# SensorsINI/v2e

Hardware: AMD Instinct MI355X
Metric: Mevents/s (EventEmulator.generate_events, 346x260, 10x slowdown) (higher is better)
Workload: dtype f64

## Files before the change

v2e_amd/csrc/emu_chain.h:

```cpp
#pragma once
#include <type_traits>
#include "pull_index.h"

#ifndef V2E_CHAIN_LOCKSTEP
#define V2E_CHAIN_LOCKSTEP 0
#endif
#ifndef V2E_CHAIN_STAMPS
#define V2E_CHAIN_STAMPS 0
#endif

constexpr int CHAIN_K_MAX = 64;
constexpr int CFRAME_THREADS = 1024;
constexpr int CHAIN_SUB = 8;
constexpr int CHAIN_MAX_ITERS = 1024;

template <typename R> __device__ __forceinline__ R floor_div_pos(R a, R b)
{
    if (!(b > (R)0) || !(a >= (R)0)) return div_floor<R>(a, b);
    if (a < b) return (R)0;
    R q = floor(a / b);
    R r = fma(-q, b, a);
    if (r < (R)0) q -= (R)1;
    else if (r >= b) q += (R)1;
    return q;
}

__device__ __forceinline__ bool clip_barrier(unsigned *ctr, unsigned target, bool light = false)
{
    __shared__ int s_ok;
    asm volatile("s_waitcnt vmcnt(0)" ::: "memory");
    __syncthreads();
    if (threadIdx.x == 0) {
        if (!light) {
            __builtin_amdgcn_fence(__ATOMIC_RELEASE, "agent");
            asm volatile("s_waitcnt vmcnt(0)" ::: "memory");
        }
        __hip_atomic_fetch_add(ctr, 1u, __ATOMIC_RELAXED, __HIP_MEMORY_SCOPE_AGENT);
        unsigned spins = 0;
        int ok = 1;
        while (__hip_atomic_load(ctr, __ATOMIC_RELAXED, __HIP_MEMORY_SCOPE_AGENT) < target) {
            if (light) __builtin_amdgcn_s_sleep(1); else __builtin_amdgcn_s_sleep(4);
            if (++spins > 2000000u) { ok = 0; break; }
        }
        if (!light) __builtin_amdgcn_fence(__ATOMIC_ACQUIRE, "agent");
        s_ok = ok;
    }
    __syncthreads();
    return s_ok != 0;
}

struct FrameTab {
    float start, step, end;
    uint32_t refr_mask;
    __device__ __forceinline__ FrameTab(const FrameCtl *c, int lane)
        : start(c->ts_start[lane & 31]), step(c->ts_stepf[lane & 31]), end(c->ts_end), refr_mask(c->refr_mask) {}
};

__device__ __forceinline__ TsGen frame_tsgen(const KArgs &a, const FrameCtl *c, const FrameTab &ft, int n, bool &use_refr)
{
    if (n <= 32) {
        use_refr = a.has_refr && ((ft.refr_mask >> (n - 1)) & 1u);
        return TsGen(__uint_as_float(lane_value(__float_as_uint(ft.start), n - 1)), ft.end,
                     __uint_as_float(lane_value(__float_as_uint(ft.step), n - 1)), n);
    }
    const double t_prev = c->t_prev, t_frame = c->t_frame;
    use_refr = a.has_refr && a.refr > (t_frame - t_prev) / (double)n;
    FrameCtl cc;
    cc.t_prev = t_prev; cc.t_frame = t_frame;
    return TsGen(cc, n, nullptr);
}

typedef float v2e_f4 __attribute__((ext_vector_type(4)));
typedef unsigned int v2e_u4 __attribute__((ext_vector_type(4)));
typedef unsigned int v2e_u2 __attribute__((ext_vector_type(2)));

__device__ __forceinline__ double lane_value_d(double v, int idx)
{
    const unsigned long long u = (unsigned long long)__double_as_longlong(v);
    return __longlong_as_double((long long)(((unsigned long long)lane_value((uint32_t)(u >> 32), idx) << 32) | lane_value((uint32_t)u, idx)));
}
__device__ __forceinline__ void store_event_wt(float4 *ev_clip, unsigned long long row, float t, float x, float y, float pol)
{
    if (row < 0x7000000ull) {
        const __amdgpu_buffer_rsrc_t r = __builtin_amdgcn_make_buffer_rsrc((void *)ev_clip, 0, 0x7fffffff, 0x00020000);
        const v2e_f4 v = {t, x, y, pol};
        __builtin_amdgcn_raw_buffer_store_b128(v, r, (int)(row * 16ull), 0, 17);
    } else {
        ev_clip[row] = make_float4(t, x, y, pol);
    }
}

struct ChainArgs {
    const void *const *frames_pp;
    unsigned long long frame_stride;
    const uint32_t *fidx_base;
    const FrameCtl *ctl;
    int f0, nf;
    int pf0, pnf;
    int D, n_clips, K, ngroups;
    int slot_f0, slot_pf0;
    uint32_t *cnt;
    uint32_t *ruleM;
    float *tsold;
    const uint2 *rec;
    uint32_t *gM_prev, *gM_cur;
    unsigned *bar_prev;
    const void *base_in, *lp_in;
    const float *ts_in;
    void *base_out, *lp_out;
    float *ts_out;
    const void *base_pin, *lp_pin;
    const float *ts_pin;
    void *base_fix, *lp_fix;
    float *ts_fix;
    void *ckc_base, *ckc_lp;
    float *ckc_ts;
    void *ckp_base, *ckp_lp;
    float *ckp_ts;
    v2e_frame_rec *recs;
    int store_out;
    int prio;
    int bar_light;
    int lockstep;
    unsigned long long *dbg;
    unsigned long long *const *stamp_pp;
    int lidx;
};

#define WT_STORE(ptr, val) __hip_atomic_store((ptr), (val), __ATOMIC_RELAXED, __HIP_MEMORY_SCOPE_SYSTEM)

#define V2E_STAMP_C(i) do { if (V2E_CHAIN_STAMPS && ca.dbg && tid == 0) ca.dbg[(size_t)g * 16 + (i)] = wall_clock64(); } while (0)

template <typename FT>
__device__ __forceinline__ void frame_record_table(const KArgs &a, FT px, const float *s_lutL, const double *s_lutI, double dt_over_tau,
                                                   double &L, double &inten01, double &eps)
{
    constexpr bool U8 = sizeof(FT) == 1;
    if (U8) {
        L = a.log_input ? (double)px : (double)s_lutL[(int)px];
        inten01 = s_lutI[(int)px];
    } else {
        const double x = (double)px;
        L = a.log_input ? x : (double)lin_log(x);
        inten01 = a.use_inten ? (x + 20.0) / 275.0 : 0.0;
    }
    eps = 0.0;
    if (a.has_cutoff) {
        eps = inten01 * dt_over_tau;
        if (eps > 1.0) eps = 1.0;
    }
}

__device__ __forceinline__ void frame_record_rand(const KArgs &a, double inten01, double shot_base, float dtime_f, float lk, float thp,
                                                  float ppre, float npre, float rr, float uu, float &dl, uint32_t &sb)
{
    dl = 0.f;
    if (a.do_leak) {
        const float rate = lk * (1.0f - a.jit_f * rr);
        dl = (dtime_f * rate) * thp;
    }
    sb = 0;
    if (a.do_shot) {
        const double F = shot_base * (a.inten_slope * inten01 + 1);
        if ((double)uu > 1 - F * (double)ppre) sb |= 1u;
        if ((double)uu < F * (double)npre) sb |= 2u;
    }
}

__device__ __forceinline__ uint4 pack_frame_record(double eps, double L, uint32_t dl_bits, uint32_t sb)
{
    const unsigned long long eb = (unsigned long long)__double_as_longlong(eps);
    uint4 r;
    r.x = (uint32_t)eb;
    r.y = (uint32_t)(eb >> 32) | (sb << 30);
    r.z = __float_as_uint((float)L);
    r.w = dl_bits;
    return r;
}

template <typename FT>
__device__ __forceinline__ uint4 make_frame_record(const KArgs &a, FT px, const float *s_lutL, const double *s_lutI, double dt_over_tau,
                                                   double shot_base, float dtime_f, float lk, float thp, float ppre, float npre, float rr,
                                                   float uu)
{
    double L, inten01, eps;
    frame_record_table<FT>(a, px, s_lutL, s_lutI, dt_over_tau, L, inten01, eps);
    float dl;
    uint32_t sb;
    frame_record_rand(a, inten01, shot_base, dtime_f, lk, thp, ppre, npre, rr, uu, dl, sb);
    return pack_frame_record(eps, L, __float_as_uint(dl), sb);
}

__device__ __forceinline__ uint4 decode_frame_record(const KArgs &a, uint2 r8, const float *s_lutL, const double *s_lutI, double dt_over_tau)
{
    const int px = (int)(r8.y & 0xFFu);
    const float tl = s_lutL[px];
    const double inten01 = s_lutI[px];
    const double L = a.log_input ? (double)px : (double)tl;
    double eps = 0.0;
    if (a.has_cutoff) {
        eps = inten01 * dt_over_tau;
        if (eps > 1.0) eps = 1.0;
    }
    return pack_frame_record(eps, L, r8.x, r8.y >> 30);
}

struct AheadArgs {
    const void *const *frames_pp;
    unsigned long long frame_stride;
    const FrameCtl *ctl;
    const uint32_t *fidx_base;
    int f0, nf, D, n_clips;
    int slot0;
    int ppt;
    uint2 *rec;
};

template <typename FT>
__global__ __launch_bounds__(BLOCK) void k_ahead(KArgs a, AheadArgs aa)
{
    static_assert(sizeof(FT) == 1, "k_ahead's records carry the pixel byte: uint8 frames only");
    __shared__ double s_lutI[256];
    const int tid = threadIdx.x;
    s_lutI[tid] = a.lut_I[tid];
    __syncthreads();
    const int clip = blockIdx.y, p = blockIdx.x * BLOCK + tid;
    if (p >= a.npx) return;
    const uint32_t fbase = *aa.fidx_base;
    const char *const frames = (const char *)*aa.frames_pp;
    const size_t sp = (size_t)clip * a.npx_pad + p;
    const bool need_r = a.do_leak && a.jit_f != 0.f;
    const float thp = a.pos_thres[sp], thn = a.neg_thres[sp];
    const float lk = a.do_leak ? a.leak_hz_f * a.noise_rate[sp] : 0.f;
    const float ppre = a.scalar_thres ? a.pos_pre_scalar : a.pos_nom_f / thp;
    const float npre = a.scalar_thres ? a.neg_pre_scalar : a.neg_nom_f / thn;
    v2e_philox_keys ks;
    v2e_philox_key_schedule((uint32_t)a.seed, (uint32_t)(a.seed >> 32), &ks);
    for (int zz = 0; zz < aa.ppt; ++zz) {
        const uint32_t q = v2e_frame_pair(fbase + (uint32_t)aa.f0) + blockIdx.z * (uint32_t)aa.ppt + (uint32_t)zz;
        const int f_odd = (int)(2u * q - 1u - fbase);
        const bool in0 = f_odd >= aa.f0 && f_odd < aa.f0 + aa.nf, in1 = f_odd + 1 >= aa.f0 && f_odd + 1 < aa.f0 + aa.nf;
        if (!in0 && !in1) continue;
        float r_odd = 0.f, u_odd = 0.f, r_even = 0.f, u_even = 0.f;
        if (need_r || a.do_shot) v2e_draw_pair_ks(&ks, (uint32_t)clip, q, (uint32_t)p, need_r, &r_odd, &u_odd, &r_even, &u_even);
#pragma unroll
        for (int half = 0; half < 2; ++half) {
            if (!(half ? in1 : in0)) continue;
            const int f = f_odd + half;
            int sl = aa.slot0 + (f - aa.f0);
            if (sl >= aa.D) sl -= aa.D;
            const FrameCtl *c = aa.ctl + (f * aa.n_clips + clip);
            const FT px = ((const FT *)(frames + (size_t)f * aa.frame_stride))[(size_t)clip * a.npx + p];
            float dl;
            uint32_t sb;
            frame_record_rand(a, s_lutI[px], c->shot_base, (float)(c->t_frame - c->t_prev), lk, thp, ppre, npre, half ? r_even : r_odd,
                              half ? u_even : u_odd, dl, sb);
            aa.rec[((uint32_t)sl * (uint32_t)aa.n_clips + (uint32_t)clip) * (uint32_t)a.npx_pad + (uint32_t)p] =
                make_uint2(__float_as_uint(dl), (uint32_t)px | (sb << 30));
        }
    }
}

template <typename R> __device__ __forceinline__ R floor_div_rcp(R a, R b, R rb)
{
    R q = floor(a * rb);
    R r = fma(-q, b, a);
    const bool lo = r < (R)0, hi = r >= b;
    q = lo ? q - (R)1 : (hi ? q + (R)1 : q);
    r = lo ? r + b : (hi ? r - b : r);
    if (__builtin_expect(!(r >= (R)0 && r < b), 0)) return floor_div_pos<R>(a, b);
    return q;
}

template <typename R, typename FT, bool FUSED, bool ALLON = false>
__global__ __launch_bounds__(BLOCK)
__attribute__((amdgpu_waves_per_eu((FUSED && sizeof(R) == 8 && sizeof(FT) == 1) ? 5 : (FUSED ? 1 : 2), 8)))
void k_chain(KArgs a_in, ChainArgs ca)
{
    KArgs a = a_in;
    if (ALLON) { a.has_cutoff = 1; a.do_leak = 1; a.do_shot = 1; a.has_refr = 1; a.use_inten = 1; }
    __shared__ float s_lutL[256];
    __shared__ double s_lutI[256];
    __shared__ double s_dtau[FUSED ? CHAIN_K_MAX : 1], s_shot[FUSED ? CHAIN_K_MAX : 1];
    __shared__ float s_dtime[FUSED ? CHAIN_K_MAX : 1];
    constexpr bool U8 = sizeof(FT) == 1;
    const int tid = threadIdx.x, lane = tid & (WAVE - 1);
    const int g = blockIdx.x;
    const int p = g * BLOCK + tid;
    const bool valid = p < a.npx;
    if (ca.prio) __builtin_amdgcn_s_setprio(3);
    V2E_STAMP_C(0);
    unsigned long long *const stamp = *ca.stamp_pp;
    if (stamp && tid == 0) atomicMax(stamp + 2 * ca.lidx, ~wall_clock64());
    uint32_t fbase = 0u;
    const char *frames = nullptr;
    float tab_L = 0.f;
    double tab_I = 0.0;
    if (!FUSED) {
        tab_L = a.lut_L[tid];
        tab_I = a.lut_I[tid];
    }
    if (FUSED) {
        fbase = *ca.fidx_base;
        frames = (const char *)*ca.frames_pp;
        if (U8) {
// ... 764 lines not shown
            uint32_t lane_tot = 0;
#pragma unroll
            for (int j = 0; j < 16; ++j) lane_tot += v[j];
            uint32_t run = carry + wave_excl_scan_u32(lane_tot, lane);
            carry += wave_sum_u32(lane_tot);
            if (wi < hi) {
                uint32_t o[16];
#pragma unroll
                for (int j = 0; j < 16; ++j) { o[j] = run; run += v[j]; }
                uint4 *dst = (uint4 *)(pre + (size_t)k * ea.nwp + wi);
                if (ea.cpre16) ea.cpre16[(((size_t)z * ea.n_clips + clip) * a.nkeys_cap + k) * (ea.nwp / 16) + wi / 16] = o[0];
                dst[0] = make_uint4(o[0], o[1], o[2], o[3]);
                dst[1] = make_uint4(o[4], o[5], o[6], o[7]);
                dst[2] = make_uint4(o[8], o[9], o[10], o[11]);
                dst[3] = make_uint4(o[12], o[13], o[14], o[15]);
            }
        }
        if (tid == 0) cT[k] = total;
    }
    __syncthreads();
    if (tid == 0) {
        __builtin_amdgcn_fence(__ATOMIC_RELEASE, "agent");
        const unsigned old = __hip_atomic_fetch_add(ea.cdone + zc, 1u, __ATOMIC_RELAXED, __HIP_MEMORY_SCOPE_AGENT);
        s_last = old == gridDim.x - 1;
        if (s_last) {
            __builtin_amdgcn_fence(__ATOMIC_ACQUIRE, "agent");
            __hip_atomic_store(ea.cdone + zc, 0u, __ATOMIC_RELAXED, __HIP_MEMORY_SCOPE_AGENT);
        }
    }
    __syncthreads();
    if (!s_last) return;
    if (discard) {
        if (tid == 0) {
            cf->M = M; cf->n_events = 0u; cf->n_signal = 0u; cf->discarded = 1u;
            rec->max_events = M;
            atomicOr(&rec->flags, V2E_FLAG_ITERS_CLAMPED);
        }
        return;
    }
    for (int k = tid; k < nk; k += CFRAME_THREADS) s_T[k] = __hip_atomic_load(cT + k, __ATOMIC_RELAXED, __HIP_MEMORY_SCOPE_AGENT);
    __syncthreads();
    if (wave != 0) return;
    uint32_t *ckb = ea.ckbase + zc * a.nkeys_cap;
    uint32_t carry = 0, sum_on = 0, sum_off = 0;
    for (int kb = 0; kb < nk; kb += WAVE) {
        const int key = kb + lane;
        const uint32_t T_k = key < nk ? s_T[key] : 0u;
        const uint32_t sig = key >= 2 ? T_k : 0u;
        const uint32_t kbase = carry + wave_excl_scan_u32(sig, lane);
        if (key < nk) ckb[key] = kbase;
        sum_on += wave_sum_u32((lane & 1) ? 0u : sig);
        sum_off += wave_sum_u32((lane & 1) ? sig : 0u);
        carry += wave_sum_u32(sig);
    }
    const uint32_t n_signal = carry;
    uint32_t *perm = ea.cperm + zc * a.max_iters * 8;
    if (a.shuffle && a.rng_mode == V2E_RNG_PHILOX) {
        const uint32_t fbase = ea.fidx_base ? *ea.fidx_base : 0u;
        for (int i = lane; i < M; i += WAVE) {
            uint32_t pk[4], sh, aa, amask;
            const uint32_t n_i = s_T[2 + 2 * i] + s_T[3 + 2 * i];
            v2e_perm_shape(n_i, &sh, &aa, &amask);
            v2e_perm_keys(a.seed, (uint32_t)clip, fbase + (uint32_t)fe, (uint32_t)i, pk);
            uint4 *pp = (uint4 *)(perm + (size_t)i * 8);
            pp[0] = make_uint4(pk[0], pk[1], pk[2], pk[3]);
            pp[1] = make_uint4(sh, aa, amask, n_i);
        }
    }
    if (lane == 0) {
        const uint32_t son = a.do_shot ? s_T[0] : 0u, soff = a.do_shot ? s_T[1] : 0u;
        cf->M = M; cf->n_signal = n_signal; cf->n_events = n_signal + son + soff; cf->discarded = 0u;
        rec->max_events = M;
        rec->n_signal = n_signal;
        rec->n_events = n_signal + son + soff;
        rec->n_on = sum_on + son;
        rec->n_off = sum_off + soff;
    }
}

__global__ __launch_bounds__(WAVE) void k_coff(CEmitArgs ea)
{
    const int clip = blockIdx.x, lane = threadIdx.x;
    unsigned long long tot = 0;
    for (int z = lane; z < ea.nE; z += WAVE) tot += ea.cf[(size_t)z * ea.n_clips + clip].n_events;
    const uint32_t lo = wave_sum_u32((uint32_t)(tot & 0xFFFFFFu)), hi = wave_sum_u32((uint32_t)(tot >> 24));
    if (lane == 0) ea.off_out[clip] = ea.off_in[clip] + lo + ((unsigned long long)hi << 24);
}

__global__ __launch_bounds__(BLOCK) void k_cemit(KArgs a, CEmitArgs ea)
{
    extern __shared__ uint32_t s_crec[];
    const int tid = threadIdx.x, lane = tid & (WAVE - 1), wave = tid / WAVE;
    const int clip = blockIdx.y, z = blockIdx.z, fe = ea.f0 + z;
    const int slot = ea.slot0 + z >= ea.D ? ea.slot0 + z - ea.D : ea.slot0 + z;
    const int grp = blockIdx.x * (BLOCK / WAVE) + wave;
    if (grp >= ea.nwaves) return;
    const size_t zc = (size_t)z * ea.n_clips + clip;
    const CFrame *cf = ea.cf + zc;
    const int p0 = grp * GROUP_PX + lane;
    const size_t sp0 = ((size_t)slot * ea.n_clips + clip) * a.npx_pad + p0;
    v2e_frame_rec *rec = ea.recs + (size_t)fe * ea.n_clips;
    const FrameCtl *c = ea.ctl + (size_t)fe * ea.n_clips + clip;
    const uint32_t *cT = ea.cT + zc * a.nkeys_cap, *ckb = ea.ckbase + zc * a.nkeys_cap;
    const uint32_t *pre = ea.cpre + zc * a.nkeys_cap * ea.nwp + grp;
    const uint32_t *perm = ea.cperm + zc * a.max_iters * 8;
    const bool shuf = (a.rng_mode == V2E_RNG_PHILOX) && a.shuffle;
    const int ICH = ea.ich;
    const uint32_t off_lo = (uint32_t)ea.off_in[clip], off_hi = (uint32_t)(ea.off_in[clip] >> 32);
    const uint32_t nj = lane < z ? ea.cf[(size_t)lane * ea.n_clips + clip].n_events : 0u;
    const int M_v = cf->M;
    const uint32_t nsig_v = cf->n_signal, nev_v = cf->n_events, disc_v = cf->discarded;
    uint32_t cw[GPX];
#pragma unroll
    for (int j = 0; j < GPX; ++j) cw[j] = p0 + j * WAVE < a.npx ? ea.cnt[sp0 + j * WAVE] : 0u;
    const int wm_v = (int)ea.wmax[zc * ea.nwp + grp];
    const FrameTab ftb(c, lane);
    uint32_t T_0 = 0, kbase_0 = 0, P_0 = 0;
    if (lane < 2 * ICH && 2 + lane < a.nkeys_cap) {
        T_0 = cT[2 + lane];
        kbase_0 = ckb[2 + lane];
        P_0 = pre[(size_t)(2 + lane) * ea.nwp];
    }
    uint4 pa_0 = make_uint4(0u, 0u, 0u, 0u), pb_0 = make_uint4(0u, 1u, 0u, 0u);
    if (shuf && lane < ICH && lane < a.max_iters) {
        pa_0 = ((const uint4 *)(perm + (size_t)lane * 8))[0];
        pb_0 = ((const uint4 *)(perm + (size_t)lane * 8))[1];
    }
    __builtin_amdgcn_sched_barrier(0);
    unsigned long long ev0 = ((unsigned long long)off_hi << 32 | off_lo) + (unsigned long long)wave_sum_u32(nj & 0xFFFFFFu) +
                             ((unsigned long long)wave_sum_u32(nj >> 24) << 24);
    const int M = __builtin_amdgcn_readfirstlane(M_v);
    const uint32_t n_signal = __builtin_amdgcn_readfirstlane((int)nsig_v);
    const uint32_t n_events = __builtin_amdgcn_readfirstlane((int)nev_v);
    if (grp == 0 && lane == 0) {
        rec[clip].ev_offset = ev0;
        if (ea.coff_in_cemit && z == ea.nE - 1) ea.off_out[clip] = ev0 + n_events;
        if (ev0 + n_events > ea.cap || n_events > 0x7FFFFFFu) atomicOr(&rec[clip].flags, V2E_FLAG_EVENTS_DROPPED);
    }
    if (__builtin_amdgcn_readfirstlane((int)disc_v)) return;
    const int wmw = __builtin_amdgcn_readfirstlane(wm_v);
    unsigned long long so[GPX], sf[GPX];
    unsigned long long any_shot = 0ull;
#pragma unroll
    for (int j = 0; j < GPX; ++j) {
        so[j] = __ballot((cw[j] & CNT_SHOT_ON) != 0);
        sf[j] = __ballot((cw[j] & CNT_SHOT_OFF) != 0);
        any_shot |= so[j] | sf[j];
    }
    if (wmw == 0 && any_shot == 0ull) return;
    const int n = M > 0 ? M : 1;
    bool use_refr;
    const TsGen tg = frame_tsgen(a, c, ftb, n, use_refr);
    int mag[GPX];
    bool neg[GPX];
    unsigned long long negb[GPX];
    float tsm[GPX];
#pragma unroll
    for (int j = 0; j < GPX; ++j) {
        mag[j] = (int)(cw[j] & CNT_MASK);
        neg[j] = (cw[j] & CNT_NEG) != 0;
        negb[j] = __ballot(neg[j]);
        tsm[j] = 0.f;
    }
    if (use_refr && ea.tsold) {
#pragma unroll
        for (int j = 0; j < GPX; ++j)
            if (p0 + j * WAVE < a.npx) tsm[j] = ea.tsold[sp0 + j * WAVE];
    }
    const uint32_t ev0_lo = (uint32_t)__builtin_amdgcn_readfirstlane((int)(uint32_t)ev0), ev0_hi = (uint32_t)__builtin_amdgcn_readfirstlane((int)(uint32_t)(ev0 >> 32));
    const unsigned long long ev0u = ((unsigned long long)ev0_hi << 32) | ev0_lo;
    const unsigned long long room = ev0u < ea.cap ? ea.cap - ev0u : 0ull;
    const unsigned long long frows = room < (unsigned long long)n_events ? room : (unsigned long long)n_events;
    const uint32_t fbytes = frows > 0x7FFFFFFull ? 0x7FFFFFF0u : (uint32_t)frows * 16u;
    const __amdgpu_buffer_rsrc_t ev_rsrc = __builtin_amdgcn_make_buffer_rsrc((void *)(ea.events + (size_t)clip * ea.cap + ev0u), 0, (int)fbytes, 0x00020000);
    auto store_row = [&](const uint32_t rel, const float t, const float x, const float y, const float pol) __attribute__((always_inline)) {
        const v2e_f4 v = {t, x, y, pol};
        __builtin_amdgcn_raw_buffer_store_b128(v, ev_rsrc, (int)(rel * 16u), 0, 17);
    };
    const unsigned long long lt = (1ull << lane) - 1ull;
    const float rcpW = 1.0f / (float)a.W;
    auto pixel_xy = [&](const uint32_t p, float &x, float &y) __attribute__((always_inline)) {
        uint32_t q;
        if (a.npx < (1 << 24)) {
            q = (uint32_t)((float)p * rcpW);
            if (q * (uint32_t)a.W > p) --q;
            else if ((q + 1u) * (uint32_t)a.W <= p) ++q;
        } else {
            q = p / (uint32_t)a.W;
        }
        y = (float)q;
        x = (float)(p - q * (uint32_t)a.W);
    };
    uint32_t *rec_w = s_crec + (size_t)wave * (ea.capw + WAVE);
    const int iters = min(wmw, M);
    for (int i0 = 0; i0 < iters; i0 += ICH) {
        const int i1 = min(i0 + ICH, iters);
        const int key = 2 + 2 * i0 + lane;
        const bool key_on = lane < 2 * ICH && key < 2 + 2 * i1;
        uint32_t T_k = 0, kbase_k = 0, P_k = 0;
        uint4 pa = make_uint4(0u, 0u, 0u, 0u), pb = make_uint4(0u, 1u, 0u, 0u);
        if (i0 == 0) {
            if (key_on) { T_k = T_0; kbase_k = kbase_0; P_k = P_0; }
            if (shuf && lane < ICH && lane < i1) { pa = pa_0; pb = pb_0; }
        } else {
            if (key_on) {
                T_k = cT[key];
                kbase_k = ckb[key];
                P_k = pre[(size_t)key * ea.nwp];
            }
            if (shuf && lane < ICH && i0 + lane < i1) {
                pa = ((const uint4 *)(perm + (size_t)(i0 + lane) * 8))[0];
                pb = ((const uint4 *)(perm + (size_t)(i0 + lane) * 8))[1];
            }
        }
        uint32_t nrec = 0;
        bool alive = true;
        for (int i = i0; i < i1; ++i) {
            unsigned long long cb[GPX], cand_any = 0ull;
#pragma unroll
            for (int j = 0; j < GPX; ++j) { cb[j] = __ballot(mag[j] > i); cand_any |= cb[j]; }
            if (cand_any == 0ull) { alive = false; break; }
            uint32_t run_on = 0, run_off = 0;
#pragma unroll
            for (int j = 0; j < GPX; ++j) {
                if (!use_refr && cb[j] == 0ull) continue;
                const bool cand = mag[j] > i;
                bool pass = cand;
                unsigned long long bo, bf;
                if (use_refr) {
                    const float t = tg(i);
                    const float pt = (cand ? 1.0f : 0.0f) * t - tsm[j];
                    pass = pt > a.refr_f;
                    if (pass) tsm[j] = t;
                    bo = __ballot(pass && !neg[j]);
                    bf = __ballot(pass && neg[j]);
                } else {
                    bf = cb[j] & negb[j];
                    bo = cb[j] & ~negb[j];
                }
                {
                    const uint32_t rank = neg[j] ? run_off + (uint32_t)__popcll(bf & lt) : run_on + (uint32_t)__popcll(bo & lt);
                    const uint32_t pos = pass ? nrec + (uint32_t)__popcll((bo | bf) & lt) : (uint32_t)(ea.capw + lane);
                    rec_w[pos] = (uint32_t)(j * WAVE + lane) | ((uint32_t)(i - i0) << GROUP_SRC_BITS) | ((neg[j] ? 1u : 0u) << (GROUP_SRC_BITS + 5)) |
                                 (rank << (GROUP_SRC_BITS + 6));
                }
                nrec += (uint32_t)__popcll(bo | bf);
                run_on += (uint32_t)__popcll(bo);
                run_off += (uint32_t)__popcll(bf);
            }
        }
        for (uint32_t e0 = 0; e0 < nrec; e0 += WAVE) {
            const bool has = e0 + lane < nrec;
            const uint32_t r = has ? rec_w[e0 + lane] : 0u;
            const uint32_t src = r & ((1u << GROUP_SRC_BITS) - 1u);
            const int il = (int)((r >> GROUP_SRC_BITS) & 31u);
            const bool eneg = (r >> (GROUP_SRC_BITS + 5)) & 1u;
            const uint32_t rank = r >> (GROUP_SRC_BITS + 6);
            const int kl = 2 * il;
            const uint32_t it_base = (uint32_t)__shfl((int)kbase_k, kl);
            const uint32_t tot_on = (uint32_t)__shfl((int)T_k, kl);
            const uint32_t off = (uint32_t)__shfl((int)P_k, kl + (eneg ? 1 : 0));
            float ex, ey;
            pixel_xy((uint32_t)(grp * GROUP_PX) + src, ex, ey);
            uint32_t cidx = (eneg ? tot_on : 0u) + off + rank;
            if (shuf) {
                v2e_perm_t pm;
                pm.k[0] = (uint32_t)__shfl((int)pa.x, il); pm.k[1] = (uint32_t)__shfl((int)pa.y, il);
                pm.k[2] = (uint32_t)__shfl((int)pa.z, il); pm.k[3] = (uint32_t)__shfl((int)pa.w, il);
                pm.sh = (uint32_t)__shfl((int)pb.x, il); pm.a = (uint32_t)__shfl((int)pb.y, il);
                pm.amask = 0u; pm.n = (uint32_t)__shfl((int)pb.w, il);
                pm.rmask = (1u << pm.sh) - 1u;
                if (has) cidx = v2e_perm_apply(&pm, cidx);
            }
            if (has) store_row(it_base + cidx, tg(i0 + il), ex, ey, eneg ? -1.0f : 1.0f);
        }
        if (!alive) break;
    }
    if (a.do_shot && any_shot) {
        const uint32_t son_tot = cT[0];
        uint32_t son_off = n_signal + pre[0], soff_off = n_signal + son_tot + pre[(size_t)ea.nwp];
        const float tl = tg(n - 1);
#pragma unroll
        for (int j = 0; j < GPX; ++j) {
            if ((so[j] | sf[j]) != 0ull) {
                float fx, fy;
                pixel_xy((uint32_t)(p0 + j * WAVE), fx, fy);
                if (cw[j] & CNT_SHOT_ON) store_row(son_off + (uint32_t)__popcll(so[j] & lt), tl, fx, fy, 1.0f);
                if (cw[j] & CNT_SHOT_OFF) store_row(soff_off + (uint32_t)__popcll(sf[j] & lt), tl, fx, fy, -1.0f);
                son_off += (uint32_t)__popcll(so[j]);
                soff_off += (uint32_t)__popcll(sf[j]);
            }
        }
    }
}

static_assert(GPX == 4, "k_cpull selects a pixel of a 256-pixel group (v2e_nth_set_bit_256)");
#ifndef V2E_PULL_ROWS
#define V2E_PULL_ROWS 8
#endif
#ifndef V2E_PULL_ROWS_TWO
#define V2E_PULL_ROWS_TWO 4
#endif
template <bool TWO>
__global__ __launch_bounds__(BLOCK) void k_cpull(KArgs a, CEmitArgs ea)
{
    constexpr int PULL_ROWS = TWO ? V2E_PULL_ROWS_TWO : V2E_PULL_ROWS;
    extern __shared__ uint32_t s_pre[];
    uint16_t *const s_idx = (uint16_t *)(s_pre + 2 * ea.p2);
    const int tid = threadIdx.x, lane = tid & (WAVE - 1);
    const int clip = blockIdx.y;
    const int blk = (int)blockIdx.x >> 3;
    const int z = (blk / ea.wpf) * 8 + ((int)blockIdx.x & 7), q = blk % ea.wpf;
    if (z >= ea.nE) return;
    const int fe = ea.f0 + z;
    const size_t zc = (size_t)z * ea.n_clips + clip;
    const CFrame *cf = ea.cf + zc;
    v2e_frame_rec *rec = ea.recs + (size_t)fe * ea.n_clips;
    const FrameCtl *c = ea.ctl + (size_t)fe * ea.n_clips + clip;
    const uint32_t *cT = ea.cT + zc * a.nkeys_cap, *ckb = ea.ckbase + zc * a.nkeys_cap;
    const uint32_t *pre = ea.cpre + zc * a.nkeys_cap * ea.nwp;
    const uint32_t *perm = ea.cperm + zc * a.max_iters * 8;
    const uint32_t *cmask = ea.cmask + zc * a.nkeys_cap * ea.nwp * (2 * GPX);
    const bool shuf = (a.rng_mode == V2E_RNG_PHILOX) && a.shuffle;
    const uint32_t off_lo = (uint32_t)ea.off_in[clip], off_hi = (uint32_t)(ea.off_in[clip] >> 32);
    const uint32_t nj = lane < z ? ea.cf[(size_t)lane * ea.n_clips + clip].n_events : 0u;
    const int M = __builtin_amdgcn_readfirstlane(cf->M);
    const uint32_t n_signal = (uint32_t)__builtin_amdgcn_readfirstlane((int)cf->n_signal);
    const uint32_t n_events = (uint32_t)__builtin_amdgcn_readfirstlane((int)cf->n_events);
    const uint32_t disc = (uint32_t)__builtin_amdgcn_readfirstlane((int)cf->discarded);
    const FrameTab ftb(c, lane);
    const unsigned long long ev0 = ((unsigned long long)off_hi << 32 | off_lo) + (unsigned long long)wave_sum_u32(nj & 0xFFFFFFu) +
                                   ((unsigned long long)wave_sum_u32(nj >> 24) << 24);
    if (q == 0 && tid == 0) {
        rec[clip].ev_offset = ev0;
        if (ea.coff_in_cemit && z == ea.nE - 1) ea.off_out[clip] = ev0 + n_events;
        if (ev0 + n_events > ea.cap || n_events > 0x7FFFFFFu) atomicOr(&rec[clip].flags, V2E_FLAG_EVENTS_DROPPED);
    }
    if (disc) return;
    const int n = M > 0 ? M : 1;
    bool use_refr;
    const TsGen tg = frame_tsgen(a, c, ftb, n, use_refr);
    const uint32_t ev0_lo = (uint32_t)__builtin_amdgcn_readfirstlane((int)(uint32_t)ev0), ev0_hi = (uint32_t)__builtin_amdgcn_readfirstlane((int)(uint32_t)(ev0 >> 32));
    const unsigned long long ev0u = ((unsigned long long)ev0_hi << 32) | ev0_lo;
    const unsigned long long room = ev0u < ea.cap ? ea.cap - ev0u : 0ull;
    unsigned long long frows64 = room < (unsigned long long)n_events ? room : (unsigned long long)n_events;
    if (frows64 > 0x7FFFFFFull) frows64 = 0x7FFFFFFull;
    const uint32_t frows = (uint32_t)frows64;
    const uint32_t per = ((frows + (uint32_t)ea.wpf - 1u) / (uint32_t)ea.wpf + (uint32_t)WAVE - 1u) & ~(uint32_t)(WAVE - 1);
    const uint32_t lo = (uint32_t)q * per, hi = min(lo + per, frows);
    if (lo >= hi) return;
    const __amdgpu_buffer_rsrc_t ev_rsrc = __builtin_amdgcn_make_buffer_rsrc((void *)(ea.events + (size_t)clip * ea.cap + ev0u), 0, (int)(frows * 16u), 0x00020000);
    const float rcpW = 1.0f / (float)a.W;
    const int P2 = ea.p2;
    bool staged = false;
    for (int i = 0; i <= M; ++i) {
        if (i == M && !a.do_shot) break;
        const int key0 = i < M ? 2 + 2 * i : 0;
        const uint32_t base = i < M ? ckb[key0] : n_signal;
        const uint32_t T_on = cT[key0], T_off = cT[key0 + 1];
        const uint32_t r_lo = max(lo, base), r_hi = min(hi, base + T_on + T_off);
        if (r_lo >= r_hi) continue;
        const uint32_t sh_on = pull_bucket_shift(T_on, (uint32_t)P2), sh_off = pull_bucket_shift(T_off, (uint32_t)P2);
        if (staged) __syncthreads();
        if (TWO) {
            const int nc16 = ea.nwp / 16;
            const uint32_t *pre16 = ea.cpre16 + (zc * a.nkeys_cap + key0) * nc16;
            for (int k = tid; k < 2 * P2; k += BLOCK) {
                const int kk = k & (P2 - 1);
                s_pre[k] = kk < nc16 ? pre16[(size_t)(k >= P2 ? nc16 : 0) + kk] : 0xFFFFFFFFu;
            }
        } else {
            for (int k = tid * 4; k < 2 * P2; k += BLOCK * 4) {
                const int kk = k & (P2 - 1), h = k >= P2 ? 1 : 0;
                const uint32_t *src = pre + (size_t)(key0 + h) * ea.nwp;
                uint4 v = make_uint4(0xFFFFFFFFu, 0xFFFFFFFFu, 0xFFFFFFFFu, 0xFFFFFFFFu);
                uint32_t nx = 0xFFFFFFFFu;
                if (kk < ea.nwp) v = *(const uint4 *)(src + kk);
                if (kk + 4 < ea.nwp) nx = src[kk + 4];
                *(uint4 *)(s_pre + k) = v;
                const uint32_t T = h ? T_off : T_on, sh = h ? sh_off : sh_on;
                uint16_t *ix = s_idx + h * P2;
                pull_index_group(ix, (uint32_t)kk, v.x, v.y, T, sh);
                pull_index_group(ix, (uint32_t)kk + 1u, v.y, v.z, T, sh);
                pull_index_group(ix, (uint32_t)kk + 2u, v.z, v.w, T, sh);
                pull_index_group(ix, (uint32_t)kk + 3u, v.w, nx, T, sh);
            }
        }
        __syncthreads();
        staged = true;
        v2e_perm_t pm;
        const bool sh_i = shuf && i < M;
        if (sh_i) {
            const uint32_t *pp = perm + (size_t)i * 8;
            pm.k[0] = pp[0]; pm.k[1] = pp[1]; pm.k[2] = pp[2]; pm.k[3] = pp[3];
            pm.sh = pp[4]; pm.a = pp[5]; pm.amask = 0u; pm.n = pp[7];
            pm.rmask = (1u << pm.sh) - 1u;
        }
        const float t = tg(i < M ? i : n - 1);
        for (uint32_t row0 = r_lo + (uint32_t)tid; row0 < r_hi; row0 += PULL_ROWS * BLOCK) {
            uint32_t gv[PULL_ROWS], rv[PULL_ROWS];
            bool nv[PULL_ROWS];
            uint4 ma[PULL_ROWS], mb[PULL_ROWS];
#pragma unroll
            for (int u = 0; u < PULL_ROWS; ++u) {
                const uint32_t row = row0 + (uint32_t)(u * BLOCK);
                if (row >= r_hi) continue;
                const uint32_t jj = row - base;
                const uint32_t ci = sh_i ? v2e_perm_invert(&pm, jj) : jj;
                const bool eneg = ci >= T_on;
                const uint32_t cp = eneg ? ci - T_on : ci;
                const uint32_t *tab = s_pre + (eneg ? P2 : 0);
                uint32_t g = 0, gbase = 0;
                if (!TWO) {
                    g = pull_index_find(tab, s_idx + (eneg ? P2 : 0), eneg ? sh_off : sh_on, cp, &gbase);
                } else {
                    for (int st = P2 >> 1; st >= 1; st >>= 1) {
                        const uint32_t v = tab[g + st];
                        if (v <= cp) g += st;
                    }
                    const uint4 *lp = (const uint4 *)(pre + (size_t)(key0 + (eneg ? 1 : 0)) * ea.nwp + g * 16u);
                    const uint4 q0 = lp[0], q1 = lp[1], q2 = lp[2], q3 = lp[3];
                    const bool h8 = q2.x <= cp;
                    const uint4 a0 = h8 ? q2 : q0, a1 = h8 ? q3 : q1;
                    const bool h4 = a1.x <= cp;
                    const uint4 b = h4 ? a1 : a0;
                    const bool h2 = b.z <= cp;
                    const uint32_t c0 = h2 ? b.z : b.x, c1 = h2 ? b.w : b.y;
                    const bool h1 = c1 <= cp;
                    gbase = h1 ? c1 : c0;
                    g = g * 16u + (h8 ? 8u : 0u) + (h4 ? 4u : 0u) + (h2 ? 2u : 0u) + (h1 ? 1u : 0u);
                }
                const uint4 *mp = (const uint4 *)(cmask + ((size_t)(key0 + (eneg ? 1 : 0)) * ea.nwp + g) * (2 * GPX));
                ma[u] = mp[0];
                mb[u] = mp[1];
                gv[u] = g;
                rv[u] = cp - gbase;
                nv[u] = eneg;
            }
#pragma unroll
            for (int u = 0; u < PULL_ROWS; ++u) {
                const uint32_t row = row0 + (uint32_t)(u * BLOCK);
                if (row >= r_hi) continue;
                const uint32_t bit = v2e_nth_set_bit_256((unsigned long long)ma[u].x | ((unsigned long long)ma[u].y << 32), (unsigned long long)ma[u].z | ((unsigned long long)ma[u].w << 32),
                                                         (unsigned long long)mb[u].x | ((unsigned long long)mb[u].y << 32), (unsigned long long)mb[u].z | ((unsigned long long)mb[u].w << 32),
                                                         rv[u]);
                const uint32_t p = gv[u] * (uint32_t)GROUP_PX + bit;
                uint32_t qy, qx;
                if (a.npx < (1 << 24)) {
                    qy = (uint32_t)((float)p * rcpW);
                    int r = (int)(p - qy * (uint32_t)a.W);
                    if (r < 0) { --qy; r += a.W; }
                    else if (r >= a.W) { ++qy; r -= a.W; }
                    qx = (uint32_t)r;
                } else {
                    qy = p / (uint32_t)a.W;
                    qx = p - qy * (uint32_t)a.W;
                }
                const v2e_f4 v = {t, (float)qx, (float)qy, nv[u] ? -1.0f : 1.0f};
                __builtin_amdgcn_raw_buffer_store_b128(v, ev_rsrc, (int)(row * 16u), 0, 19);
            }
        }
    }
}
```

Before: 20140.

## Restructure pull kernel rows into wave-uniform batched trips with lockstep searches

Rewrites the k_cpull row loop as a lambda over compile-time row batches with a wave-uniform trip count, so per-row bounds checks become a single clamp and the tail is handled by 4/2/1-row trips. The permutation inversion, the shared-memory binary search and the nth-set-bit selection are rewritten as branch-free lockstep loops that exit on wave-wide __any, with perm keys scalarised via readfirstlane. It also adds a 32-bit-word nth-set-bit, a branchless divide fix-up, and an occupancy hint on the TWO variant. The aim is to cut divergence and scalar overhead in the event-emission pull kernel, at the cost of higher register pressure and extra iterations for lanes that finish early.

```diff
diff --git a/v2e_amd/csrc/emu_chain.h b/v2e_amd/csrc/emu_chain.h
--- a/v2e_amd/csrc/emu_chain.h
+++ b/v2e_amd/csrc/emu_chain.h
@@ -1,6 +1,7 @@
 #pragma once
 #include <type_traits>
 #include "pull_index.h"
+#include "pull_select.h"
 
 #ifndef V2E_CHAIN_LOCKSTEP
 #define V2E_CHAIN_LOCKSTEP 0
@@ -1371,7 +1372,7 @@
 #define V2E_PULL_ROWS_TWO 4
 #endif
 template <bool TWO>
-__global__ __launch_bounds__(BLOCK) void k_cpull(KArgs a, CEmitArgs ea)
+__device__ __forceinline__ void cpull_rows(KArgs a, CEmitArgs ea)
 {
     constexpr int PULL_ROWS = TWO ? V2E_PULL_ROWS_TWO : V2E_PULL_ROWS;
     extern __shared__ uint32_t s_pre[];
@@ -1457,37 +1458,88 @@
         }
         __syncthreads();
         staged = true;
-        v2e_perm_t pm;
         const bool sh_i = shuf && i < M;
+        uint32_t pk0 = 0, pk1 = 0, pk2 = 0, pk3 = 0, psh = 0, pa = 0, pn = 0;
         if (sh_i) {
             const uint32_t *pp = perm + (size_t)i * 8;
-            pm.k[0] = pp[0]; pm.k[1] = pp[1]; pm.k[2] = pp[2]; pm.k[3] = pp[3];
-            pm.sh = pp[4]; pm.a = pp[5]; pm.amask = 0u; pm.n = pp[7];
-            pm.rmask = (1u << pm.sh) - 1u;
-        }
+            pk0 = (uint32_t)__builtin_amdgcn_readfirstlane((int)pp[0]); pk1 = (uint32_t)__builtin_amdgcn_readfirstlane((int)pp[1]);
+            pk2 = (uint32_t)__builtin_amdgcn_readfirstlane((int)pp[2]); pk3 = (uint32_t)__builtin_amdgcn_readfirstlane((int)pp[3]);
+            psh = (uint32_t)__builtin_amdgcn_readfirstlane((int)pp[4]); pa = (uint32_t)__builtin_amdgcn_readfirstlane((int)pp[5]);
+            pn = (uint32_t)__builtin_amdgcn_readfirstlane((int)pp[7]);
+        }
+        const uint32_t prmask = (1u << psh) - 1u;
         const float t = tg(i < M ? i : n - 1);
-        for (uint32_t row0 = r_lo + (uint32_t)tid; row0 < r_hi; row0 += PULL_ROWS * BLOCK) {
-            uint32_t gv[PULL_ROWS], rv[PULL_ROWS];
-            bool nv[PULL_ROWS];
-            uint4 ma[PULL_ROWS], mb[PULL_ROWS];
-#pragma unroll
-            for (int u = 0; u < PULL_ROWS; ++u) {
-                const uint32_t row = row0 + (uint32_t)(u * BLOCK);
-                if (row >= r_hi) continue;
-                const uint32_t jj = row - base;
-                const uint32_t ci = sh_i ? v2e_perm_invert(&pm, jj) : jj;
-                const bool eneg = ci >= T_on;
-                const uint32_t cp = eneg ? ci - T_on : ci;
-                const uint32_t *tab = s_pre + (eneg ? P2 : 0);
-                uint32_t g = 0, gbase = 0;
-                if (!TWO) {
-                    g = pull_index_find(tab, s_idx + (eneg ? P2 : 0), eneg ? sh_off : sh_on, cp, &gbase);
-                } else {
+        const uint32_t *const cm_i = cmask + (size_t)key0 * ea.nwp * (2 * GPX);
+        const uint32_t *const pre_i = pre + (size_t)key0 * ea.nwp;
+        auto trip = [&](const uint32_t row0, auto rc) {
+            constexpr int R = decltype(rc)::value;
+            uint32_t ci[R], cpv[R], kov[R], gv[R], rv[R];
+            float pol[R];
+            uint4 ma[R], mb[R];
+#pragma unroll
+            for (int u = 0; u < R; ++u) {
+                uint32_t row = row0 + (uint32_t)(u * BLOCK);
+                if (u == R - 1) row = min(row, r_hi - 1u);
+                ci[u] = row - base;
+            }
+            if (sh_i) {
+#pragma unroll
+                for (int u = 0; u < R; ++u) ci[u] = pull_perm_rounds(pk0, pk1, pk2, pk3, pa, psh, prmask, ci[u]);
+                for (;;) {
+                    bool pend = false;
+                    uint32_t xs = 0;
+                    int su = -1;
+                    for (int u = 0; u < R; ++u) {
+                        const bool pu = ci[u] >= pn;
+                        pend |= pu;
+                        xs = pu ? ci[u] : xs;
+                        su = pu ? u : su;
+                    }
+                    if (!__any(pend)) break;
+                    const uint32_t xr = pull_perm_rounds(pk0, pk1, pk2, pk3, pa, psh, prmask, xs);
+                    for (int u = 0; u < R; ++u) ci[u] = su == u ? xr : ci[u];
+                }
+            }
+            if (!TWO) {
+                uint32_t lo[R], hi[R];
+#pragma unroll
+                for (int u = 0; u < R; ++u) {
+                    const bool eneg = ci[u] >= T_on;
+                    cpv[u] = eneg ? ci[u] - T_on : ci[u];
+                    kov[u] = eneg ? (uint32_t)P2 : 0u;
+                    pol[u] = eneg ? -1.0f : 1.0f;
+                    const uint32_t bk = kov[u] + (cpv[u] >> (eneg ? sh_off : sh_on));
+                    lo[u] = s_idx[bk];
+                    hi[u] = s_idx[bk + 1u];
+                }
+                for (;;) {
+                    bool more = false;
+                    for (int u = 0; u < R; ++u) more |= lo[u] < hi[u];
+                    if (!__any(more)) break;
+                    for (int u = 0; u < R; ++u) {
+                        const uint32_t mid = pull_find_mid(lo[u], hi[u]);
+                        pull_find_step(&lo[u], &hi[u], mid, s_pre[kov[u] + mid], cpv[u]);
+                    }
+                }
+#pragma unroll
+                for (int u = 0; u < R; ++u) {
+                    gv[u] = lo[u];
+                    rv[u] = cpv[u] - s_pre[kov[u] + lo[u]];
+                }
+            } else {
+#pragma unroll
+                for (int u = 0; u < R; ++u) {
+                    const bool eneg = ci[u] >= T_on;
+                    const uint32_t cp = eneg ? ci[u] - T_on : ci[u];
+                    kov[u] = eneg ? (uint32_t)P2 : 0u;
+                    pol[u] = eneg ? -1.0f : 1.0f;
+                    const uint32_t *tab = s_pre + kov[u];
+                    uint32_t g = 0;
                     for (int st = P2 >> 1; st >= 1; st >>= 1) {
                         const uint32_t v = tab[g + st];
                         if (v <= cp) g += st;
                     }
-                    const uint4 *lp = (const uint4 *)(pre + (size_t)(key0 + (eneg ? 1 : 0)) * ea.nwp + g * 16u);
+                    const uint4 *lp = (const uint4 *)(pre_i + (eneg ? (uint32_t)ea.nwp : 0u) + g * 16u);
                     const uint4 q0 = lp[0], q1 = lp[1], q2 = lp[2], q3 = lp[3];
                     const bool h8 = q2.x <= cp;
                     const uint4 a0 = h8 ? q2 : q0, a1 = h8 ? q3 : q1;
@@ -1496,38 +1548,58 @@
                     const bool h2 = b.z <= cp;
                     const uint32_t c0 = h2 ? b.z : b.x, c1 = h2 ? b.w : b.y;
                     const bool h1 = c1 <= cp;
-                    gbase = h1 ? c1 : c0;
-                    g = g * 16u + (h8 ? 8u : 0u) + (h4 ? 4u : 0u) + (h2 ? 2u : 0u) + (h1 ? 1u : 0u);
-                }
-                const uint4 *mp = (const uint4 *)(cmask + ((size_t)(key0 + (eneg ? 1 : 0)) * ea.nwp + g) * (2 * GPX));
+                    gv[u] = g * 16u + (h8 ? 8u : 0u) + (h4 ? 4u : 0u) + (h2 ? 2u : 0u) + (h1 ? 1u : 0u);
+                    rv[u] = cp - (h1 ? c1 : c0);
+                }
+            }
+#pragma unroll
+            for (int u = 0; u < R; ++u) {
+                const uint4 *mp = (const uint4 *)(cm_i + ((kov[u] ? (uint32_t)ea.nwp : 0u) + gv[u]) * (uint32_t)(2 * GPX));
                 ma[u] = mp[0];
                 mb[u] = mp[1];
-                gv[u] = g;
-                rv[u] = cp - gbase;
-                nv[u] = eneg;
-            }
-#pragma unroll
-            for (int u = 0; u < PULL_ROWS; ++u) {
+            }
+            uint32_t pv[R];
+#pragma unroll
+            for (int u = 0; u < R; ++u)
+                pv[u] = gv[u] * (uint32_t)GROUP_PX + pull_nth_set_bit_8x32(ma[u].x, ma[u].y, ma[u].z, ma[u].w, mb[u].x, mb[u].y, mb[u].z, mb[u].w, rv[u]);
+            auto store = [&](const int u, const uint32_t qx, const uint32_t qy) {
                 const uint32_t row = row0 + (uint32_t)(u * BLOCK);
-                if (row >= r_hi) continue;
-                const uint32_t bit = v2e_nth_set_bit_256((unsigned long long)ma[u].x | ((unsigned long long)ma[u].y << 32), (unsigned long long)ma[u].z | ((unsigned long long)ma[u].w << 32),
-                                                         (unsigned long long)mb[u].x | ((unsigned long long)mb[u].y << 32), (unsigned long long)mb[u].z | ((unsigned long long)mb[u].w << 32),
-                                                         rv[u]);
-                const uint32_t p = gv[u] * (uint32_t)GROUP_PX + bit;
-                uint32_t qy, qx;
-                if (a.npx < (1 << 24)) {
-                    qy = (uint32_t)((float)p * rcpW);
-                    int r = (int)(p - qy * (uint32_t)a.W);
-                    if (r < 0) { --qy; r += a.W; }
-                    else if (r >= a.W) { ++qy; r -= a.W; }
-                    qx = (uint32_t)r;
-                } else {
-                    qy = p / (uint32_t)a.W;
-                    qx = p - qy * (uint32_t)a.W;
-                }
-                const v2e_f4 v = {t, (float)qx, (float)qy, nv[u] ? -1.0f : 1.0f};
-                __builtin_amdgcn_raw_buffer_store_b128(v, ev_rsrc, (int)(row * 16u), 0, 19);
-            }
-        }
-    }
-}
+                const v2e_f4 v = {t, (float)qx, (float)qy, pol[u]};
+                if (u < R - 1 || row < r_hi)
+                    __builtin_amdgcn_raw_buffer_store_b128(v, ev_rsrc, (int)(row * 16u), 0, 19);
+            };
+            if (a.npx < (1 << 24)) {
+#pragma unroll
+                for (int u = 0; u < R; ++u) {
+                    uint32_t qy, qx;
+                    pull_div_fix(pv[u], (uint32_t)a.W, (uint32_t)((float)pv[u] * rcpW), &qy, &qx);
+                    store(u, qx, qy);
+                }
+            } else {
+#pragma unroll
+                for (int u = 0; u < R; ++u) {
+                    const uint32_t qy = pv[u] / (uint32_t)a.W;
+                    store(u, pv[u] - qy * (uint32_t)a.W, qy);
+                }
+            }
+        };
+        const uint32_t wrow0 = r_lo + (uint32_t)__builtin_amdgcn_readfirstlane(tid - lane);
+        uint32_t cnt = wrow0 < r_hi ? (r_hi - wrow0 + (uint32_t)BLOCK - 1u) / (uint32_t)BLOCK : 0u;
+        uint32_t row0 = r_lo + (uint32_t)tid;
+        for (; cnt >= (uint32_t)PULL_ROWS; cnt -= (uint32_t)PULL_ROWS, row0 += (uint32_t)(PULL_ROWS * BLOCK))
+            trip(row0, std::integral_constant<int, PULL_ROWS>());
+        if (PULL_ROWS > 4 && (cnt & 4u)) {
+            trip(row0, std::integral_constant<int, 4>());
+            row0 += (uint32_t)(4 * BLOCK);
+        }
+        if (PULL_ROWS > 2 && (cnt & 2u)) {
+            trip(row0, std::integral_constant<int, 2>());
+            row0 += (uint32_t)(2 * BLOCK);
+        }
+        if (cnt & 1u) trip(row0, std::integral_constant<int, 1>());
+    }
+}
+template <bool TWO>
+__global__ __launch_bounds__(BLOCK) void k_cpull(KArgs a, CEmitArgs ea) { cpull_rows<TWO>(a, ea); }
+template <>
+__global__ __launch_bounds__(BLOCK, 6) void k_cpull<true>(KArgs a, CEmitArgs ea) { cpull_rows<true>(a, ea); }
diff --git a/v2e_amd/csrc/pull_select.h b/v2e_amd/csrc/pull_select.h
--- /dev/null
+++ b/v2e_amd/csrc/pull_select.h
@@ -0,0 +1,84 @@
+#pragma once
+#include <stdint.h>
+#ifndef __cplusplus
+#include <stdbool.h>
+#endif
+#include "../../include/v2e_detmath.h"
+
+#if defined(__HIPCC__)
+#define V2E_PS_HD __host__ __device__ __forceinline__
+#else
+#define V2E_PS_HD static inline
+#endif
+
+V2E_PS_HD uint32_t pull_bfe(uint32_t v, uint32_t pos, uint32_t width)
+{
+#if defined(__HIP_DEVICE_COMPILE__)
+    return __builtin_amdgcn_ubfe(v, pos, width);
+#else
+    return (v >> (pos & 31u)) & ((1u << width) - 1u);
+#endif
+}
+
+V2E_PS_HD uint32_t pull_nth_set_bit_8x32(uint32_t d0, uint32_t d1, uint32_t d2, uint32_t d3, uint32_t d4, uint32_t d5, uint32_t d6,
+                                         uint32_t d7, uint32_t r)
+{
+    const uint32_t p0 = (uint32_t)__builtin_popcount(d0), p1 = (uint32_t)__builtin_popcount(d1) + p0,
+                   p2 = (uint32_t)__builtin_popcount(d2) + p1, p3 = (uint32_t)__builtin_popcount(d3) + p2,
+                   p4 = (uint32_t)__builtin_popcount(d4) + p3, p5 = (uint32_t)__builtin_popcount(d5) + p4,
+                   p6 = (uint32_t)__builtin_popcount(d6) + p5;
+    const bool h2 = r >= p3;
+    uint32_t w0 = h2 ? d4 : d0, w1 = h2 ? d5 : d1;
+    const uint32_t w2 = h2 ? d6 : d2, w3 = h2 ? d7 : d3;
+    uint32_t acc = h2 ? p3 : 0u, q0 = h2 ? p4 : p0;
+    const uint32_t q1 = h2 ? p5 : p1, q2 = h2 ? p6 : p2;
+    const bool h1 = r >= q1;
+    w0 = h1 ? w2 : w0;
+    w1 = h1 ? w3 : w1;
+    acc = h1 ? q1 : acc;
+    q0 = h1 ? q2 : q0;
+    const bool h0 = r >= q0;
+    w0 = h0 ? w1 : w0;
+    acc = h0 ? q0 : acc;
+    uint32_t pos = (h2 ? 128u : 0u) | (h1 ? 64u : 0u) | (h0 ? 32u : 0u);
+#if defined(__HIPCC__)
+#pragma unroll
+#endif
+    for (int k = 4; k >= 0; --k) {
+        const uint32_t s = 1u << k;
+        const uint32_t cs = (uint32_t)__builtin_popcount(pull_bfe(w0, pos, s)) + acc;
+        const bool up = r >= cs;
+        acc = up ? cs : acc;
+        pos = up ? pos | s : pos;
+    }
+    return pos;
+}
+
+V2E_PS_HD uint32_t pull_perm_rounds(uint32_t k0, uint32_t k1, uint32_t k2, uint32_t k3, uint32_t a, uint32_t sh, uint32_t rmask,
+                                    uint32_t x)
+{
+    uint32_t l = x >> sh, r = x & rmask;
+    r = (r - v2e_mix32(l + k3)) & rmask;
+    uint32_t f = (uint32_t)(((uint64_t)v2e_mix32(r + k2) * a) >> 32);
+    l = l >= f ? l - f : l + (a - f);
+    r = (r - v2e_mix32(l + k1)) & rmask;
+    f = (uint32_t)(((uint64_t)v2e_mix32(r + k0) * a) >> 32);
+    l = l >= f ? l - f : l + (a - f);
+    return (l << sh) | r;
+}
+
+V2E_PS_HD uint32_t pull_find_mid(uint32_t lo, uint32_t hi) { return (lo + hi + 1u) >> 1; }
+V2E_PS_HD void pull_find_step(uint32_t *lo, uint32_t *hi, uint32_t mid, uint32_t v, uint32_t cp)
+{
+    const bool le = v <= cp;
+    *lo = le ? mid : *lo;
+    *hi = le ? *hi : mid - 1u;
+}
+
+V2E_PS_HD void pull_div_fix(uint32_t p, uint32_t W, uint32_t qy, uint32_t *y, uint32_t *x)
+{
+    const int32_t r = (int32_t)(p - qy * W);
+    const bool lt = r < 0, ge = r >= (int32_t)W;
+    *y = qy + (ge ? 1u : 0u) - (lt ? 1u : 0u);
+    *x = (uint32_t)(r + (lt ? (int32_t)W : 0) - (ge ? (int32_t)W : 0));
+}
```

After: 20480, median of 6. +1.7%, better.
